# nipponjo/tts-arabic-pytorch

Measured on AMD Instinct MI355X. Metric: audio samples/sec (FastPitch+HiFi-GAN, synthetic 64-phoneme inputs), higher is better.
Workload: dtype f32

## Files before the change

tts-arabic-pytorch_amd/csrc/api.hip:

```cpp
#include <cerrno>
#include <cstdio>
#include <cstdlib>
#include <cstring>
#include <algorithm>
#include <atomic>
#include <mutex>
#include <string>
#include <vector>

#include "kernels.hpp"

namespace ttsamd {

static thread_local std::string g_err;

void set_error(const char* fmt, ...) {
    char buf[1024];
    va_list ap;
    va_start(ap, fmt);
    vsnprintf(buf, sizeof(buf), fmt, ap);
    va_end(ap);
    g_err = buf;
}

// ... 205 lines not shown
    unsigned v = __float_as_uint(r);
    v += 0x7fffu + ((v >> 16) & 1u);
    out[i] = (unsigned short)h;
    out[n + i] = (unsigned short)(v >> 16);
}

namespace {
struct OptDesc { const char* name; int kind; long long lo, hi; };
const OptDesc kOpts[OPT_COUNT] = {
#define TTS_OPT_DESC(name, kind, lo, hi) {"TTSAMD_" #name, kind, lo, hi},
    TTS_OPTIONS(TTS_OPT_DESC)
#undef TTS_OPT_DESC
};
std::atomic<const char*> g_opt[OPT_COUNT];
std::once_flag g_opt_once;
std::string g_opt_env_error;

bool opt_valid(const OptDesc& d, const char* v) {
    if (!v || !*v) return false;
    char* end = nullptr;
    errno = 0;
    const long long x = std::strtoll(v, &end, d.kind == 1 ? 16 : 10);
    if (!(errno == 0 && end != v && *end == '\0' && x >= d.lo && x <= d.hi)) return false;
    if (&d == &kOpts[OPT_WINO4] && (((x & 32) && !(x & 2)) || ((x & 64) && !(x & 4)) || ((x & 128) && !(x & 8)))) return false;
    return true;
}
void opt_init() {
    std::call_once(g_opt_once, [] {
        for (int i = 0; i < OPT_COUNT; ++i) {
            const char* e = std::getenv(kOpts[i].name);
            if (!e || !*e) continue;
            if (!opt_valid(kOpts[i], e)) {
                if (g_opt_env_error.empty()) {
                    char buf[256];
                    std::snprintf(buf, sizeof buf, "%s='%s' in the environment is not a valid value (%s in [%llx, %llx])", kOpts[i].name, e,
                                  kOpts[i].kind == 1 ? "hex mask" : "integer", kOpts[i].lo, kOpts[i].hi);
                    g_opt_env_error = buf;
                }
                continue;
            }
            g_opt[i].store(strdup(e), std::memory_order_release);
        }
    });
}
int opt_find(const char* name) {
    if (!name) return -1;
    for (int i = 0; i < OPT_COUNT; ++i)
// ... 844 lines not shown
```

tts-arabic-pytorch_amd/csrc/common.hpp:

```cpp
#pragma once
#include <hip/hip_runtime.h>
#include <stdint.h>
#include <atomic>
#include <cstdarg>
#include <cstdio>
#include <cstdlib>
#include <string>

#include "../../include/ttsamd.h"

namespace ttsamd {

void set_error(const char* fmt, ...);

#define TTS_CHECK_HIP(expr)                                                         \
    do {                                                                            \
        hipError_t e_ = (expr);                                                     \
        if (e_ != hipSuccess) {                                                     \
            ttsamd::set_error("%s failed: %s (%s:%d)", #expr, hipGetErrorString(e_), \
                              __FILE__, __LINE__);                                  \
            return TTSAMD_EHIP;                                                     \
        }                                                                           \
    } while (0)

// ... 7 lines not shown

#define TTS_TRY(expr)               \
    do {                            \
        int32_t rc_ = (expr);       \
        if (rc_ != 0) return rc_;   \
    } while (0)

inline int64_t align_up(int64_t x, int64_t a) { return (x + a - 1) / a * a; }

inline hipError_t lds_opt_in(const void* fn, int bytes, std::atomic<uint64_t>& done) {
    int dev = 0;
    hipError_t e = hipGetDevice(&dev);
    if (e != hipSuccess) return e;
    if (dev >= 0 && dev < 64 && ((done.load(std::memory_order_acquire) >> dev) & 1)) return hipSuccess;
    e = hipFuncSetAttribute(fn, hipFuncAttributeMaxDynamicSharedMemorySize, bytes);
    if (e == hipSuccess && dev >= 0 && dev < 64) done.fetch_or(1ull << dev, std::memory_order_release);
    return e;
}

#define TTS_OPTIONS(X)                                                                                     \
    X(HIFIGAN_STREAMS, 0, 0, 1)    \
    X(WINO, 0, 0, 1)                                              \
    X(WINO2, 0, 0, 31)             \
    X(WINO4, 0, 0, 255)            \
    X(FUSED_PAIR, 0, 0, 1)                   \
    X(FUSED2, 0, 0, 1)                                           \
    X(FUSED2_MASK, 1, 0, 0x1ff)               \
    X(FUSED2_MASK_N1, 1, 0, 0x1ff)          \
    X(FUSED2_WB, 0, 0, 2)                     \
    X(PAIR4, 0, 0, 2)              \
    X(CONVT, 0, 0, 1)                              \
    X(CONVT_WINO, 0, 0, 2)         \
    X(BFO, 0, 0, 1)                \
    X(BFO_CHAIN, 0, 0, 1)                           \
    X(BFO_CHAIN7, 0, 0, 1)                                 \
    X(BFO_FF, 0, 0, 1)                              \
    X(BFO_SPLITK, 0, 0, 1)                                              \
    X(BFO_SMALL_TILES, 0, 0, 1)            \
    X(BF16_ATTN, 0, 0, 1)                                         \
    X(BF16_PACKED_T, 0, 0, 1)                   \
    X(ATT_RA, 0, 1, 4)                             \
    X(ATT_SPLIT, 0, 0, 1)                      \
    X(XCD_W, 0, 0, 1)                            \
    X(XCD_WMAX_KB, 0, 0, 1 << 20)     \
    X(DEEP_SPLITK, 0, 0, 1)        \
    X(TACO_PERSISTENT, 0, 0, 2)    \
    X(TACO_SEG, 0, 8, 1 << 20)     \
// ... 93 lines not shown
                           int32_t mode, float div, float slope, int32_t ntw, hipStream_t stream, const float* w2_wino = nullptr,
                           const float* w1_wino = nullptr);
bool fused_pair4_supported(int32_t channels, int32_t k, int32_t dil, int32_t L, const float* x, const float* y);
int32_t launch_fused_pair4(int32_t channels, const float* x, float* y, const float* w1_wino4, const float* b1, const float* w2_wino4,
                           const float* b2, int32_t k, int32_t dil, const int64_t* lens, int32_t len_mul, int32_t L, int32_t batch,
                           int32_t mode, float div, float slope, hipStream_t stream, int32_t points = 6);
bool resblock2_conv_supported(int32_t channels, int32_t k, int32_t dil, int32_t L, const float* x, const float* y);
int32_t launch_resblock2_conv(int32_t channels, const float* x, float* y, const float* w, const float* b, int32_t k, int32_t dil,
                              const int64_t* lens, int32_t len_mul, int32_t L, int32_t batch, int32_t mode, float div, float slope,
                              hipStream_t stream);
bool resblock2_pair_supported(int32_t channels, int32_t k, int32_t d1, int32_t d2, int32_t L, const float* x, const float* y);
int32_t launch_resblock2_pair(int32_t channels, const float* x, float* y, const float* w1, const float* b1, const float* w2,
                              const float* b2, int32_t k, int32_t d1, int32_t d2, const int64_t* lens, int32_t len_mul, int32_t L,
                              int32_t batch, int32_t mode, float div, float slope, hipStream_t stream);
int wino_route(const ConvParams& p);
int32_t launch_wino(const ConvParams& p, hipStream_t stream);
void pack_wino_weight(const float* w, int cout, int cin, float* out);
int wino2_groups(int k);
int wino2_block_outputs(int coutp, int dil);
int32_t launch_wino2(const ConvParams& p, hipStream_t stream);
void pack_wino2_weight(const float* w, int cout, int cin, int k, float* out);
int wino4_groups(int k);
int wino44_groups(int k);
constexpr int kWino4Default = 255;
bool wino44_wanted(const ConvParams& p);
int wino4_block_outputs(int dil);
__host__ __device__ constexpr int wino4_pk_tuples(int n, int d) { return d * ((n + 4 * d - 1) / (4 * d)); }
__host__ __device__ constexpr int wino4_pk_tiles(int n, int d) { return (wino4_pk_tuples(n, d) + 63) / 64; }
__host__ __device__ constexpr int wino4_pk_col(int t, int d) { return (t / d) * 4 * d + t % d; }
__host__ __device__ constexpr int wino4_pk_q0(int tile, int d) { return (64 * tile / d) * 4 * d; }
__host__ __device__ constexpr int wino4_pk_r0(int tile, int d) { return 64 * tile % d; }
int wino4_ksplit(const ConvParams& p);
int32_t launch_splitk_reduce(const ConvParams& q, hipStream_t stream);
int32_t launch_wino4(const ConvParams& p, hipStream_t stream);
void wino4_filter_groups(const float* g, int k, float* o);
void pack_wino4_weight(const float* w, int cout, int cin, int k, float* out);
void wino44_filter_groups(const float* g, int k, float* o);
void pack_wino44_weight(const float* w, int cout, int cin, int k, float* out);
void pack_conv_weight(const float* w, int cout, int cin, int k, float* out);
void pack_convt_weight(const float* w, int cin, int cout, int kt, int u, int p, float* out);
inline int cout_padded(int cout) { return (int)align_up(cout, 32); }
void split_packed_bf16(const float* packed, int64_t n, uint16_t* out);
int32_t default_precision();

#ifdef __HIPCC__
template <int EXTRA = 0, bool PACKED = false>
__device__ __forceinline__ bool live_tile(const int64_t* __restrict__ lens, const int mul, const int n_max, const int tile_w,
// ... 37 lines not shown
```

tts-arabic-pytorch_amd/csrc/conv_wino4.hip:

```cpp
#include <cstdlib>
#include <cstring>

#include <algorithm>
#include <vector>

#include "conv_mfma_common.hpp"
#include "conv_row_epilogue.hpp"
#include "bfo.hpp"

namespace ttsamd {

typedef float w4_f32x4 __attribute__((ext_vector_type(4)));
typedef float w4_f32x2 __attribute__((ext_vector_type(2)));

template <int K, int NOCT_, int NSTAGE_, int PT_ = 6, int LP_ = 1, int CT_ = 0, int PK_ = 0>
struct Wino4Geo {
    static_assert(PK_ == 0 || LP_ == 2, "packed tiles: the strip kernels");
    static constexpr bool PT7 = PT_ == 7;
    static_assert(PT_ == 6 || (PT7 && (K == 7 || K == 11)), "seven-point groups: k = 7 / 11");
    static_assert(CT_ == 0 || (K == 3 && PT_ == 6 && LP_ == 1), "transposed conv: the k = 3 six-point form at dilation 1");
    static constexpr int WM = 2, WN = 2;
    static constexpr int NSF = K == 1 ? 0 : (K == 3 ? 1 : (K == 7 ? 2 : (PT7 ? 3 : 4)));
    static constexpr int NL = (!PT7 && (K == 7 || K == 1)) ? 1 : 0;
    static constexpr int GSF = PT7 ? 7 : 6;
    static constexpr int SSF = PT7 ? 4 : 3;
    static constexpr int NG = PT7 ? (K == 7 ? 13 : 20) : (K == 1 ? 4 : (K == 3 ? (CT_ ? 5 : 6) : (K == 7 ? 16 : 23)));
    static constexpr int NGQ = PT7 ? NG : ((NG + 1) & ~1);
    static constexpr bool WSHARE = K == 1;
    static constexpr int NGW = WSHARE ? 1 : NGQ;
    static constexpr int NPL = PT7 ? 7 : (NL ? 8 : (CT_ ? 5 : 6));
    static constexpr int NPOS = K == 1 ? 4 : (K == 3 ? (CT_ ? 5 : 6) : (K == 7 ? 10 : 14));
    static constexpr int NOCT = NOCT_, NSTAGE = NSTAGE_;
    static constexpr int NPH = PT7 ? ((K == 11 && LP_ == 2) ? 2 : 1) : (K == 11 ? 2 : 1);
    static constexpr int PH0 = PT7 ? 8 : 12;
    static constexpr int NGPM = NPH == 1 ? NG : 12;
    static_assert(NPH == 1 || (PH0 <= NGPM && NG - PH0 <= NGPM), "phase sizes");
    static constexpr int CO_BLK = WM * 32;
    static constexpr int NTUP = WN * 32;
    static constexpr int NT_BLK = 4 * NTUP;
    static constexpr int BUF4 = NOCT * 2 * NGPM * NTUP;
    static constexpr int PF = 4;
    static constexpr int NM = 4;
    __host__ __device__ static constexpr int glo(int ph) { return NPH == 1 ? 0 : PH0 * ph; }
// ... 13 lines not shown
    __host__ __device__ static constexpr int mlo(int ph) { return gfirst(glo(ph)); }
    __host__ __device__ static constexpr int mhi(int ph) {
        int m = 0;
        for (int g = glo(ph); g < glo(ph) + ngp(ph); ++g) m = glast(g) > m ? glast(g) : m;
        return m;
    }
    static_assert(mhi(NPH - 1) == NPOS - 1 && mlo(0) == 0, "the groups cover the window and nothing past it");
    __host__ __device__ static constexpr int npos(int ph) { return mhi(ph) - mlo(ph) + 1; }
    static constexpr int NPOSP = npos(0) > npos(NPH - 1) ? npos(0) : npos(NPH - 1);
    __host__ __device__ static constexpr int ngap(int ph) { return NOCT * ngp(ph) * NM; }
    __host__ __device__ static constexpr int sph(int ph) { return ((ph - (NSTAGE - 1)) % NPH + NPH) % NPH; }
    __host__ __device__ static constexpr int sgap(int ph) { return ngap(sph(ph)); }
    static constexpr int JSF = 10;
    __host__ __device__ static constexpr int sflo(int ph) { return glo(ph) / 7; }
    __host__ __device__ static constexpr bool inph(int ph, int g) { return g >= glo(ph) && g < glo(ph) + ngp(ph); }
    __host__ __device__ static constexpr int glast_ph(int ph) { return glo(ph) + ngp(ph) - 1; }
    __host__ __device__ static constexpr int nwj(int ph) {
        return PT7 ? JSF * (glast_ph(ph) / 7 - sflo(ph)) + (glast_ph(ph) % 7 == 0 ? 3 : JSF) : NOCT * ngp(ph);
    }
    static_assert(!PT7 || (NOCT == 1 && glo(0) % 7 <= 1 && glo(NPH - 1) % 7 <= 1 &&
                           (glast_ph(0) % 7 == 0 || glast_ph(0) % 7 >= 5) && glast_ph(NPH - 1) % 7 >= 5),
                  "seven-point phases: start on V0 / V1 of a sub-filter (the partial sums are formed per phase), end on V0 or the last row");
    __host__ __device__ static constexpr int fdiv4(int e) { return e >= 0 ? e / 4 : -((3 - e) / 4); }
    __host__ __device__ static constexpr int vlo(int ph) { return fdiv4(mlo(ph) - (K - 1) / 2); }
    __host__ __device__ static constexpr int nvec(int ph) { return fdiv4(mhi(ph) - (K - 1) / 2) - vlo(ph) + 1; }
    static constexpr int NVP = nvec(0) > nvec(NPH - 1) ? nvec(0) : nvec(NPH - 1);
    __host__ __device__ static constexpr int nljv(int ph) { return NOCT * 2 * nvec(ph); }
    static constexpr int DAV = (K == 3 || K == 1) ? 8 : 16;
    __host__ __device__ static constexpr int tw0v(int ph) { return DAV + 2 * nljv(ph); }
    __host__ __device__ static constexpr int wsv(int ph) { return (sgap(ph) - tw0v(ph)) / nwj(ph); }
    static_assert(LP_ != 1 || (wsv(0) >= 1 && wsv(NPH - 1) >= 1), "one write job per gap at most (vector loads)");
    __host__ __device__ static constexpr int strip_need(int d) {
        return 3 + (PK_ ? wino4_pk_col(d - 1 + 63, d) : wino4_pk_col(4 * 64 / (4 * d) * d - 1, d)) + (NPOS - 1) * d + 1;
    }
    static constexpr int RAWW = (PK_ && K == 11) ? 332 : 320;
    static_assert(RAWW % 4 == 0 && RAWW >= 256 && RAWW <= 512 && strip_need(3) <= RAWW && strip_need(5) <= RAWW, "the strip holds every tuple's window");
    static constexpr int NV2 = (RAWW - 256) / 4;
    static constexpr int NROW = 2 * NOCT;
    static constexpr int RAW_BYTES = 4 * (NROW * RAWW * 4 + 16);
    static constexpr int DAT = K == 7 ? 16 : (K == 11 ? 12 : 8);
    __host__ __device__ static constexpr int nrj(int ph) { return NROW * ((npos(ph) + 1) / 2); }
    __host__ __device__ static constexpr bool loads_in(int ph) { return ph == 0; }
    __host__ __device__ static constexpr int tr_r0(int ph) { return loads_in(ph) ? DAT + 2 * NROW : 0; }
    __host__ __device__ static constexpr int tw0t(int ph) { return tr_r0(ph) + nrj(ph) + 1; }
    __host__ __device__ static constexpr int wst(int ph) { return (sgap(ph) - tw0t(ph)) / nwj(ph); }
    static_assert(LP_ != 2 || (wst(0) >= 1 && wst(NPH - 1) >= 1), "one write job per gap at most (strip path)");
    static constexpr int QX = WSHARE ? 0 : (NOCT * ngq(0)) % PF;
    static constexpr int QMAIN = NOCT * ngq(0) - QX;
    static_assert(QX == 0 || (NPH == 1 && NOCT == 1 && QMAIN >= 2 * PF), "extra queue slots: one phase, one octet");
    static_assert((WSHARE ? NOCT : NOCT * ngq(NPH - 1)) % PF == 0 || QX != 0, "queue slots line up across steps");
    static_assert((size_t)NSTAGE * BUF4 * 16 + (LP_ == 2 ? RAW_BYTES : 0) <= 80 * 1024, "two blocks per CU");
    static_assert(NPH == 1 || NOCT == 1, "phases split an octet's groups");
};

// ... 19 lines not shown
        if (!wino4_pk_covers(n, d)) return false;
    return true;
}
static_assert(wino4_pk_covers_range(1, 1, 130, 1) && wino4_pk_covers_range(1, 131, 700, 13), "packed tiles, d = 1: rows of 1 .. 700 outputs");
static_assert(wino4_pk_covers_range(3, 1, 130, 1) && wino4_pk_covers_range(3, 131, 700, 13), "packed tiles, d = 3: rows of 1 .. 700 outputs");
static_assert(wino4_pk_covers_range(5, 1, 130, 1) && wino4_pk_covers_range(5, 131, 700, 13), "packed tiles, d = 5: rows of 1 .. 700 outputs");
static_assert(wino4_pk_covers_range(3, 1020, 1030, 1) && wino4_pk_covers_range(5, 1020, 1030, 1), "packed tiles: around 1028");
static_assert(wino4_pk_covers(1357, 3) && wino4_pk_covers(1357, 5) && wino4_pk_covers(2048, 3) && wino4_pk_covers(2048, 5), "packed tiles: long rows");
static_assert(wino4_pk_covers(28672, 3), "packed tiles, d = 3: a row of 28672");
static_assert(wino4_pk_covers(28672, 5), "packed tiles, d = 5: a row of 28672");
static_assert(wino4_pk_tiles(1028, 5) == 5 && wino4_pk_tuples(1028, 5) == 260 && wino4_pk_tuples(1028, 3) == 258, "packed tiles of a row of 1028");

template <int K, int NOCT_, int NSTAGE_, int EPI, int LP, int PT = 6>
__global__ __launch_bounds__(256, kConvMinWaves) void conv1d_wino4_f32(const ConvParams p) {
    extern __shared__ __attribute__((aligned(16))) float4 smem4[];
    constexpr int CTU = EPI == 5 ? 8 : (EPI == 6 ? 2 : 0);
    constexpr bool CT = CTU != 0;
    constexpr bool PK = EPI == 7;
    using G = Wino4Geo<K, NOCT_, NSTAGE_, PT, LP, CTU, PK ? 1 : 0>;
    constexpr bool PT7 = G::PT7;
    constexpr int WN = G::WN, NSF = G::NSF, NOCT = G::NOCT, NSTAGE = G::NSTAGE, NPL = G::NPL, NGPM = G::NGPM;
    constexpr int CO_BLK = G::CO_BLK, NTUP = G::NTUP, NT_BLK = G::NT_BLK, PF = G::PF;
    constexpr int NPH = G::NPH, NPOSP = G::NPOSP, NM = G::NM;
    constexpr bool D1 = LP == 1, TR = LP == 2;
    static_assert(D1 || TR, "window path");
    const int dil = D1 ? 1 : p.dil;
    const int nt_eff = wino4_tile(dil, NTUP), ntup_eff = nt_eff / 4;
    const int tiles_y = p.CoutP / CO_BLK;
    const int per_tile = tiles_y * p.ksplit;
    const unsigned sidx = blockIdx.x, xcd = sidx & 7u, u = sidx >> 3;
    const int yk = (int)(u % (unsigned)per_tile);
    const unsigned gt = (u / (unsigned)per_tile) * 8u + xcd;
    const int n_tiles_x = PK ? wino4_pk_tiles(p.Nout, dil) : (p.Nout + nt_eff - 1) / nt_eff;
    const int tile_w = PK ? 1 : nt_eff;
    int b = (int)(gt / (unsigned)n_tiles_x);
    int q0 = (int)(gt % (unsigned)n_tiles_x) * tile_w;
    if (p.compact) {
        int tile = 0;
        if (!live_tile<CT ? 1 : 0, PK>(p.lens_out, p.len_out_mul, p.Nout, nt_eff, p.batch, gt, b, tile, dil)) return;
        b = __builtin_amdgcn_readfirstlane(b);
        q0 = __builtin_amdgcn_readfirstlane(tile) * tile_w;
    } else if (b >= p.batch) {
        return;
    }
    int r0 = 0;
    if constexpr (PK) {
        r0 = wino4_pk_r0(q0, dil);
// ... 4 lines not shown
    const int ks = yk / tiles_y;
    const int co_blk0 = (yk - ks * tiles_y) * CO_BLK;
    int n_out = p.Nout;
    if constexpr (CT) {
        if (p.lens_out) {
            const int len = min(p.Lin, (int)p.lens_out[b] * p.len_out_mul);
            n_out = len > 0 ? len + 1 : 0;
        }
    } else {
        if (p.lens_out) n_out = min(n_out, (int)p.lens_out[b] * p.len_out_mul);
    }
    if (q0 >= n_out) return;
    int in_len = p.Lin;
    if (p.lens_in) in_len = min(in_len, (int)p.lens_in[b] * p.len_in_mul);

    const int x_cs = p.x_cs, CoutP = p.CoutP;
    const int chunks_all = p.Cin / (8 * NOCT);
    const int c_beg = (int)((int64_t)ks * chunks_all / p.ksplit), n_chunks = (int)((int64_t)(ks + 1) * chunks_all / p.ksplit);
    const int n_groups = (p.Cin / 8) * G::NGW;
    const float* __restrict__ xb = p.x + (int64_t)b * p.x_bs;
    const float in_slope = p.in_slope;

    constexpr bool REG = EPI >= 3, RES = EPI == 3;
    static_assert(!REG || ((LP == 1 || PK) && K != 1), "register epilogue: dilation 1 or the packed strip form, k = 3 / 7 / 11");
    static_assert(!PK || LP == 2, "packed tiles: the strip kernels");
    static_assert(EPI <= 7 && (!CT || K == 3), "epilogues 0, 3, 4, 7 and the transposed conv's 5 / 6 (k = 3 form)");
    float ep_bias = 0.f;
    if constexpr (!REG) {
        if (tid < CO_BLK && p.bias) ep_bias = p.bias[min(co_blk0 + tid, p.Cout - 1)];
    }

    const int kk = lane >> 5, l31 = lane & 31;
    const int pe = wn * 32 + l31;
    const int col_e = PK ? wino4_pk_col(r0 + pe, dil) : (dil == 1 ? 4 * pe : (pe / dil) * 4 * dil + pe % dil);
    f32x16 acc[NPL];
#pragma unroll
    for (int g = 0; g < NPL; ++g)
#pragma unroll
        for (int r = 0; r < 16; ++r) acc[g][r] = 0.f;
    const int ep_row0 = REG ? co_blk0 + __builtin_amdgcn_readfirstlane(wm) * 32 : 0;
    const int ep_voff = (q0 + col_e < n_out ? q0 + col_e : 0) * 4;
    const int ep_rrow = ep_row0 + 4 * kk;
    const bfo_i4 ep_rs = bfo_rsrc(RES ? p.res + (int64_t)b * p.r_bs : nullptr, RES ? (unsigned)p.Cout * (unsigned)p.r_cs * 4u : 0u);
    const bfo_i4 ep_bs = bfo_rsrc(p.bias, (REG && p.bias) ? (unsigned)p.Cout * 4u : 0u);
    w4_f32x4 rq[RES ? 16 : 1], bsq[REG ? 4 : 1];
    constexpr int EP_T0 = RES ? 16 : 0;
#define TTS_EPLOAD_JOB(T)                                                                            \
// ... 4 lines not shown
            bsq[REG ? (T) - EP_T0 : 0] = __builtin_bit_cast(w4_f32x4, bfo_ld16(ep_bs, (ep_rrow + 8 * ((T) - EP_T0)) * 4, 0, 0)); \
    }

    const bfo_i4 wrs = bfo_rsrc(K == 1 ? p.w : (PT7 ? p.w_wino44 : p.w_wino4), (unsigned)n_groups * 2u * (unsigned)CoutP * 16u);
    const int wv = (kk * CoutP + co_blk0 + wm * 32 + l31) * 16;
    const int wstep = 2 * CoutP * 16, wlast = (n_groups - 1) * wstep;
    int wso = c_beg * NOCT * G::NGW * wstep;
    w4_f32x4 aq[PF + G::QX];
    if constexpr (G::QX == 0) {
#pragma unroll
        for (int g = 0; g < PF; ++g) {
            aq[g] = __builtin_bit_cast(w4_f32x4, bfo_ld16(wrs, wv, wso, 0));
            wso = min(wso + wstep, wlast);
        }
    } else {
#pragma unroll
        for (int g = 0; g < PF + G::QX; ++g)
            aq[g] = __builtin_bit_cast(w4_f32x4, bfo_ld16(wrs, wv, min(wso + (g < PF ? g : G::QMAIN + g - PF) * wstep, wlast), 0));
    }

    const int sh = __builtin_amdgcn_readfirstlane((tid >> 7) & 1), skk = __builtin_amdgcn_readfirstlane((tid >> 6) & 1);
    w4_f32x2 sx[D1 ? 1 : NOCT][D1 ? 1 : NPOSP];
    w4_f32x4 sv[D1 ? NOCT : 1][2][D1 ? G::NVP : 1];
    w4_f32x2 ta[NOCT], tb[NOCT];
    w4_f32x2 tf[PT7 ? 5 : 1], te[PT7 ? 4 : 1], td[PT7 ? 3 : 1], th[PT7 ? 2 : 1];
    const int spe = PK ? r0 + lane : min(lane, ntup_eff - 1);
    const int xw0 = (q0 + 4 * lane) * 4;
    constexpr int pad_c = (K - 1) / 2;
    const int ch_off = (4 * sh + skk) * x_cs;

#define TTS_VJOB_IDX(PH, J)                                                                          \
        const int nv_ = G::nvec(PH);                                                                 \
        const int ol_ = (J) / (2 * nv_), pp_ = ((J) / nv_) % 2, vi_ = (J) % nv_;
#define TTS_VLOAD_JOB(PH, J, XSO)                                                                    \
    {                                                                                                \
        TTS_VJOB_IDX(PH, J)                                                                          \
        const bfo_i4 xrs_ = bfo_rsrc(xb + ((XSO) + ch_off + (8 * ol_ + 2 * pp_) * x_cs), (unsigned)in_len * 4u);     \
        sv[ol_][pp_][vi_] = __builtin_bit_cast(w4_f32x4, bfo_ld16(xrs_, xw0 + 16 * (G::vlo(PH) + vi_), 0, 0));      \
    }
#define TTS_VACT_JOB(PH, A)                                                                          \
    {                                                                                                \
        TTS_VJOB_IDX(PH, (A) / 2)                                                                    \
        if ((A) % 2 == 0) {                                                                          \
            sv[ol_][pp_][vi_].x = bfo_lrelu(sv[ol_][pp_][vi_].x, in_slope);                          \
            sv[ol_][pp_][vi_].y = bfo_lrelu(sv[ol_][pp_][vi_].y, in_slope);                          \
        } else {                                                                                     \
            sv[ol_][pp_][vi_].z = bfo_lrelu(sv[ol_][pp_][vi_].z, in_slope);                          \
            sv[ol_][pp_][vi_].w = bfo_lrelu(sv[ol_][pp_][vi_].w, in_slope);                          \
        }                                                                                            \
    }
    float* const strip = reinterpret_cast<float*>(smem4 + NSTAGE * G::BUF4) + wid * (G::NROW * G::RAWW + 4);
    const int tr_a = (q0 - pad_c * dil) & ~3;
    const int tr_off = q0 + (dil == 1 ? 4 * spe : (spe / dil) * 4 * dil + spe % dil) - pad_c * dil - tr_a;
    w4_f32x4 rv[TR ? G::NROW : 1][2];
#define TTS_TLOAD_JOB(J, XSO)                                                                        \
    {                                                                                                \
        const int pp_ = (J) / 2, vs_ = (J) % 2;                                                      \
        const bfo_i4 xrs_ = bfo_rsrc(xb + ((XSO) + ch_off + (8 * (pp_ / 2) + 2 * (pp_ % 2)) * x_cs), (unsigned)in_len * 4u); \
        const int v_ = lane + 64 * vs_;                                                              \
        rv[pp_][vs_] = __builtin_bit_cast(w4_f32x4, bfo_ld16(xrs_, (vs_ == 1 && lane >= G::NV2) ? BFO_OOB : (tr_a + 4 * v_) * 4, 0, 0)); \
    }
#define TTS_TSTORE_JOB(J)                                                                            \
    {                                                                                                \
        const int pp_ = (J) / 2, vs_ = (J) % 2;                                                      \
        w4_f32x4 a_ = rv[pp_][vs_];                                                                  \
        a_.x = bfo_lrelu(a_.x, in_slope); a_.y = bfo_lrelu(a_.y, in_slope);                          \
        a_.z = bfo_lrelu(a_.z, in_slope); a_.w = bfo_lrelu(a_.w, in_slope);                          \
        const int v_ = lane + 64 * vs_;                                                              \
        float* dst_ = (vs_ == 1 && lane >= G::NV2) ? strip + G::NROW * G::RAWW : strip + pp_ * G::RAWW + 4 * v_;    \
        *reinterpret_cast<w4_f32x4*>(dst_) = a_;                                                     \
    }
#define TTS_TREAD_JOB(PH, J)                                                                         \
    {                                                                                                \
        const int npr_ = (G::npos(PH) + 1) / 2;                                                      \
        const int pp_ = (J) / npr_, jp_ = (J) % npr_;                                                \
        const float* src_ = strip + pp_ * G::RAWW + tr_off + (G::mlo(PH) + 2 * jp_) * dil;           \
        sx[pp_ / 2][2 * jp_][pp_ % 2] = src_[0];                                                     \
        if (2 * jp_ + 1 < G::npos(PH)) sx[pp_ / 2][2 * jp_ + 1][pp_ % 2] = src_[dil];                \
    }
#define TTS_SXV(M) (w4_f32x2{sv[ol_][0][G::fdiv4((M) - pad_c) - G::vlo(PH_)][((M) - pad_c) - 4 * G::fdiv4((M) - pad_c)],     \
                             sv[ol_][1][G::fdiv4((M) - pad_c) - G::vlo(PH_)][((M) - pad_c) - 4 * G::fdiv4((M) - pad_c)]})
#define TTS_SX(M) (D1 ? TTS_SXV(M) : sx[D1 ? 0 : ol_][D1 ? 0 : (M) - G::mlo(PH_)])
#define TTS_WRITE_JOB(PH, J, WR)                                                                     \
    {                                                                                                \
        const int PH_ = (PH);                                                                        \
        const int ol_ = PT7 ? 0 : (J) / G::ngp(PH_), gl_ = (J) % G::ngp(PH_), g_ = G::glo(PH_) + gl_;                          \
        w4_f32x2 v2;                                                                                 \
        if constexpr (PT7) {                                                                         \
             \
            const int sf_ = G::sflo(PH_) + (J) / G::JSF, kd_ = (J) % G::JSF, s4 = 4 * sf_, g0_ = 7 * sf_;                      \
            const bool v0_ = G::inph(PH_, g0_), tap4_ = g0_ + 6 < G::NG;                             \
            int row_ = -1;                                                                           \
            if (kd_ == 0) {                         \
                if (v0_) tf[0] = sf_ > G::sflo(PH_) ? tf[4] : TTS_SX(s4 + 2) - 4.f * TTS_SX(s4);    \
                tf[1] = TTS_SX(s4 + 3) - 4.f * TTS_SX(s4 + 1);                                       \
                tf[2] = TTS_SX(s4 + 4) - 4.f * TTS_SX(s4 + 2);                                       \
            } else if (kd_ == 1) {                                                                   \
                tf[3] = TTS_SX(s4 + 5) - 4.f * TTS_SX(s4 + 3);                                       \
                if (v0_) te[0] = tf[0] - 2.f * tf[1];                                                \
            } else if (kd_ == 2) {                                                                   \
                te[2] = tf[2] - 2.f * tf[3];                                                         \
                if (v0_) { v2 = te[2] - te[0]; row_ = 0; }                                           \
            } else if (kd_ == 3) {                                                                   \
                te[1] = tf[1] - 2.f * tf[2];                                                         \
                v2 = te[1] + te[2]; row_ = 1;                                                        \
// ... 34 lines not shown
                v2 = ta[ol_] + tb[ol_];                                                              \
            } else if (i_ == 4) v2 = ta[ol_] - tb[ol_];                                              \
            else v2 = 4.f * TTS_SX(s3 + 1) + (TTS_SX(s3 + 5 < G::NPOS ? s3 + 5 : s3) - 5.f * TTS_SX(s3 + 3));           \
        } else {                                                                                     \
            v2 = TTS_SX(3 * NSF + (g_ - 6 * NSF));                                                   \
        }                                                                                            \
        if constexpr (!PT7) (WR)[2 * ((ol_ * 2 * NGPM + gl_) * NTUP)] = v2;                          \
    }

    const float4* sB = smem4 + kk * NGPM * NTUP + wn * 32 + l31;
    w4_f32x2* sW = reinterpret_cast<w4_f32x2*>(smem4 + skk * NGPM * NTUP + lane) + sh;
    float4 bq[2];

    {
#pragma unroll
        for (int st = 0; st < NSTAGE - 1; ++st) {
            const int ph = st % NPH;
            const int xso = min(c_beg + st / NPH, n_chunks - 1) * 8 * NOCT * x_cs;
            if constexpr (D1) {
#pragma unroll
                for (int J = 0; J < G::nljv(ph); ++J) TTS_VLOAD_JOB(ph, J, xso)
#pragma unroll
                for (int J = 0; J < 2 * G::nljv(ph); ++J) TTS_VACT_JOB(ph, J)
            } else {
                if (G::loads_in(ph)) {
#pragma unroll
                    for (int J = 0; J < 2 * G::NROW; ++J) TTS_TLOAD_JOB(J, xso)
#pragma unroll
                    for (int J = 0; J < 2 * G::NROW; ++J) TTS_TSTORE_JOB(J)
                }
#pragma unroll
                for (int J = 0; J < G::nrj(ph); ++J) TTS_TREAD_JOB(ph, J)
            }
            w4_f32x2* wr = sW + 2 * st * G::BUF4;
#pragma unroll
            for (int J = 0; J < G::nwj(ph); ++J) TTS_WRITE_JOB(ph, J, wr)
        }
    }
    __syncthreads();
    bq[0] = sB[0];

    int stage = 0;
#define TTS_CHUNK_STEPS(LAST, C) \
        _Pragma("unroll")                                                                                                                                    \
        for (int ph = 0; ph < NPH; ++ph) {                                                                                                                   \
            const bool peel = (LAST) && ph == NPH - 1;                                                                                                       \
// ... 20 lines not shown
                    aq[qs] = __builtin_bit_cast(w4_f32x4, bfo_ld16(wrs, wv, wso, 0));                                                                        \
                    wso = min(wso + wstep, wlast);                                                                                                           \
                }                                                                                                                                            \
                if (gl >= G::ngp(ph)) continue;                                                     \
                const int r = ol * G::ngp(ph) + gl;                                                                \
                const int cur = r & 1, nxt = cur ^ 1;                                                                                                        \
                const int plane = G::plane(G::glo(ph) + gl);                                                                                                 \
                                                    \
                if (r + 1 < NOCT * G::ngp(ph)) bq[nxt] = rd[(((r + 1) / G::ngp(ph)) * 2 * NGPM + (r + 1) % G::ngp(ph)) * NTUP];                              \
                else if (NSTAGE >= 3 && !peel) bq[nxt] = sB[sn * G::BUF4];        \
                __builtin_amdgcn_sched_barrier(0);                                                                                                           \
                const float bv[4] = {bq[cur].x, bq[cur].y, bq[cur].z, bq[cur].w};                                                                            \
        _Pragma("unroll")                                                                                                                                    \
                for (int m = 0; m < NM; ++m) {                                                                                                               \
                    acc[plane] = __builtin_amdgcn_mfma_f32_32x32x2f32(a4[m], bv[m], acc[plane], 0, 0, 0);                                                    \
                                   \
                                                                                             \
                    const int t = r * NM + m;                                                                                                                \
                    if (peel) {                                                                                                                              \
                        TTS_EPLOAD_JOB(t)                                                                                                                    \
                    } else if constexpr (D1) {                                                                                                               \
                        if (t < G::nljv(tph)) TTS_VLOAD_JOB(tph, t, xso)                                                                                     \
                        if (t >= G::DAV && t - G::DAV < 2 * G::nljv(tph)) TTS_VACT_JOB(tph, t - G::DAV)                                                      \
                        if (t >= G::tw0v(tph) && (t - G::tw0v(tph)) % G::wsv(tph) == 0 &&                                                                    \
                            (t - G::tw0v(tph)) / G::wsv(tph) < G::nwj(tph))                                                                                  \
                            TTS_WRITE_JOB(tph, (t - G::tw0v(tph)) / G::wsv(tph), wr)                                                                         \
                    } else {                                                                                                                                 \
                        if (G::loads_in(tph) && t < 2 * G::NROW) TTS_TLOAD_JOB(t, xso)                                                                       \
                        if (G::loads_in(tph) && t >= G::DAT && t < G::DAT + 2 * G::NROW) TTS_TSTORE_JOB(t - G::DAT)                                          \
                        if (t >= G::tr_r0(tph) && t - G::tr_r0(tph) < G::nrj(tph)) TTS_TREAD_JOB(tph, t - G::tr_r0(tph))                                     \
                        if (t >= G::tw0t(tph) && (t - G::tw0t(tph)) % G::wst(tph) == 0 && (t - G::tw0t(tph)) / G::wst(tph) < G::nwj(tph))                    \
                            TTS_WRITE_JOB(tph, (t - G::tw0t(tph)) / G::wst(tph), wr)                                                                         \
                    }                                                                                                                                        \
                    __builtin_amdgcn_sched_barrier(0);                                                                                                       \
                }                                                                                                                                            \
            }                                                                                                                                                \
            if (peel) break;                                                                                                                                 \
            __syncthreads();                                                                                                                                 \
            if (NSTAGE < 3) bq[0] = sB[sn * G::BUF4];                                      \
            else if ((NOCT * G::ngp(ph)) % 2 != 0) bq[0] = bq[1];                                                                                            \
            stage = stage_next;                                                                                                                              \
        }
    for (int c = c_beg; c < n_chunks - (REG ? 1 : 0); ++c) {
        TTS_CHUNK_STEPS(false, c)
    }
    if constexpr (REG) {
        const int c = n_chunks - 1;
        TTS_CHUNK_STEPS(true, c)
    }
#undef TTS_CHUNK_STEPS
#undef TTS_EPLOAD_JOB
#undef TTS_TLOAD_JOB
#undef TTS_TSTORE_JOB
#undef TTS_TREAD_JOB
#undef TTS_VLOAD_JOB
#undef TTS_VACT_JOB
#undef TTS_VJOB_IDX
#undef TTS_SXV
#undef TTS_SX
#undef TTS_WRITE_JOB

#define TTS_OUT_QUAD(R)                                                                              \
        const float s12 = acc[1][R] + acc[2][R], d12 = acc[1][R] - acc[2][R];                        \
        const float s34 = acc[3][R] + acc[4][R], d34 = acc[3][R] - acc[4][R];                        \
        float y0 = acc[0][R] + s12 + s34;                                                            \
        float y1 = d12 + 2.f * d34;                                                                  \
        float y2 = s12 + 4.f * s34;                                                                  \
        float y3 = d12 + 8.f * d34 + acc[PT7 ? 6 : 5][R];                                            \
        if constexpr (NSF == 0) { y0 = acc[0][R]; y1 = 0.f; y2 = 0.f; y3 = acc[5][R]; }               \
        if constexpr (PT7) {                                                                   \
            y0 += acc[5][R];                                                                         \
            y1 += 0.5f * acc[5][R];                                                                  \
            y2 += 0.25f * acc[5][R];                                                                 \
            y3 += 0.125f * acc[5][R];                                                                \
        } else if constexpr (NPL == 8) {                                                             \
            y1 += acc[6][R];                                                                         \
            y2 += acc[7][R];                                                                         \
        }
// ... 193 lines not shown
    static_assert(EPI < 3 || lds == ring + strip, "register epilogue: the ring (and the strip) set the LDS size");
    static std::atomic<uint64_t> lds_done{0};
    const auto kern = conv1d_wino4_f32<K, NOCT, NSTAGE, EPI, LP, PT>;
    TTS_CHECK_HIP(lds_opt_in((const void*)kern, (int)lds, lds_done));
    const int nt = wino4_tile(p.dil, G::NTUP);
    ConvParams q = p;
    q.ksplit = EPI == 0 ? wino4_ksplit(p) : 1;
    note_conv_launch(PK ? (PT == 7 ? 8 : 7) : (PT == 7 ? 4 : 3), q.ksplit);
    const int64_t n_tiles = (int64_t)(PK ? wino4_pk_tiles(p.Nout, p.dil) : (p.Nout + nt - 1) / nt) * p.batch;
    const int64_t n_blocks = ((n_tiles + 7) / 8) * 8 * (p.CoutP / G::CO_BLK) * q.ksplit;
    TTS_REQUIRE(n_blocks < ((int64_t)1 << 31), "wino4: %lld blocks", (long long)n_blocks);
    dim3 grid((unsigned)n_blocks, 1, 1);
    q.compact = compact_order(p.lens_out, p.batch) ? 1 : 0;
    hipLaunchKernelGGL(kern, grid, dim3(256), lds, stream, q);
    TTS_CHECK_HIP(hipGetLastError());
    if (q.ksplit > 1) return launch_splitk_reduce(q, stream);
    return 0;
}

static bool wino4_packed_wanted(const ConvParams& p) {
    return ((int)opt_int(OPT_WINO4, kWino4Default) & 128) != 0 && p.dil != 1 && p.res == nullptr && p.mode == 0 && wino4_ksplit(p) == 1;
}

template <int K, int NOCT, int NSTAGE>
static int32_t launch_wino4_cfg(const ConvParams& p, hipStream_t stream) {
    if (p.dil == 1) {
        if (wino4_ksplit(p) != 1) return launch_wino4_epi<K, NOCT, NSTAGE, 0, 1>(p, stream);
        if (p.res != nullptr) return launch_wino4_epi<K, NOCT, NSTAGE, 3, 1>(p, stream);
        return launch_wino4_epi<K, NOCT, NSTAGE, 4, 1>(p, stream);
    }
    if (wino4_packed_wanted(p)) return launch_wino4_epi<K, NOCT, 2, 7, 2>(p, stream);
    return launch_wino4_epi<K, NOCT, 2, 0, 2>(p, stream);
}

template <int K>
static int32_t launch_wino44_cfg(const ConvParams& p, hipStream_t stream) {
    if (p.dil == 1) {
        if (wino4_ksplit(p) != 1) return launch_wino4_epi<K, 1, 2, 0, 1, 7>(p, stream);
        if (p.res != nullptr) return launch_wino4_epi<K, 1, 2, 3, 1, 7>(p, stream);
        return launch_wino4_epi<K, 1, 2, 4, 1, 7>(p, stream);
    }
    if (wino4_packed_wanted(p)) return launch_wino4_epi<K, 1, 2, 7, 2, 7>(p, stream);
    return launch_wino4_epi<K, 1, 2, 0, 2, 7>(p, stream);
}

bool wino44_wanted(const ConvParams& p) {
    if (p.w_wino44 == nullptr || (p.K != 7 && p.K != 11)) return false;
    return ((int)opt_int(OPT_WINO4, kWino4Default) & (p.K == 7 ? 32 : 64)) != 0;
}
// ... 2 lines not shown
    if (wino44_wanted(p)) return p.K == 7 ? launch_wino44_cfg<7>(p, stream) : launch_wino44_cfg<11>(p, stream);
    if (p.K == 1) return launch_wino4_epi<1, 4, 2, 0, 1>(p, stream);
    if (p.K == 3) return launch_wino4_cfg<3, 2, 3>(p, stream);
    if (p.K == 7) return launch_wino4_cfg<7, 1, 2>(p, stream);
    if (p.K == 11) return launch_wino4_cfg<11, 1, 3>(p, stream);
    set_error("wino4: kernel size %d not built (1, 3, 7, 11)", p.K);
    return TTSAMD_EINVAL;
}

int wino4_block_outputs(int dil) { return wino4_tile(dil, 64); }

bool convt_wino_packable(int cin, int cout, int u) { return (u == 2 || u == 8) && cin >= 16 && cin % 16 == 0 && cout >= 1 && (u * cout) % 64 == 0; }

bool convt_wino_supported(const ConvParams& p, const float* w_wino, const float* bias_wino) {
    const int u = p.n_phase;
    return w_wino != nullptr && bias_wino != nullptr && p.precision == 0 && convt_wino_packable(p.Cin, p.Cout, u) && p.K == 2 && p.dil == -1 &&
           p.phase_p * 2 == u && p.y_ts == u && p.res == nullptr && p.mode == 0 && p.scale == nullptr && p.relu_out == 0 &&
           !p.x_packed && !p.y_packed && p.in_slope >= 0.f && p.in_slope <= 1.f && p.Lin == p.Nout &&
           (p.x_cs & 3) == 0 && (p.x_bs & 3) == 0 && ((uintptr_t)p.x & 15) == 0 &&
           (p.y_cs & 3) == 0 && (p.y_bs & 3) == 0 && ((uintptr_t)p.y & 15) == 0 &&
           (int64_t)p.Lin * 4 + 64 < ((int64_t)1 << 31) && (int64_t)p.Cout * p.y_cs * 4 < ((int64_t)1 << 31);
}

template <int U>
static int32_t launch_convt_wino_u(const ConvParams& p, const float* w_wino, const float* bias_wino, hipStream_t stream) {
    constexpr int EPI = U == 8 ? 5 : 6;
    using G = Wino4Geo<3, 2, 3, 6, 1, U>;
    constexpr size_t lds = (size_t)G::NSTAGE * G::BUF4 * sizeof(float4);
    static_assert(lds <= 80 * 1024, "two blocks per CU");
    static std::atomic<uint64_t> lds_done{0};
    const auto kern = conv1d_wino4_f32<3, 2, 3, EPI, 1, 6>;
    TTS_CHECK_HIP(lds_opt_in((const void*)kern, (int)lds, lds_done));
    ConvParams q = p;
    q.w_wino4 = w_wino; q.bias = bias_wino;
    q.Cout = U * p.Cout; q.CoutP = q.Cout;
    q.Nout = p.Lin + 1;
    q.K = 3; q.dil = 1; q.pad = 1; q.n_phase = 1; q.ksplit = 1;
    const int64_t n_tiles = (int64_t)((q.Nout + G::NT_BLK - 1) / G::NT_BLK) * p.batch;
    const int64_t n_blocks = ((n_tiles + 7) / 8) * 8 * (q.CoutP / G::CO_BLK);
    TTS_REQUIRE(n_blocks < ((int64_t)1 << 31), "convt wino: %lld blocks", (long long)n_blocks);
    q.compact = compact_order(p.lens_out, p.batch) ? 1 : 0;
    hipLaunchKernelGGL(kern, dim3((unsigned)n_blocks, 1, 1), dim3(256), lds, stream, q);
    TTS_CHECK_HIP(hipGetLastError());
    return 0;
}

int32_t launch_convt_wino(const ConvParams& p, const float* w_wino, const float* bias_wino, hipStream_t stream) {
    TTS_REQUIRE(convt_wino_supported(p, w_wino, bias_wino), "convt wino: unsupported geometry");
    if (p.Nout <= 0) return 0;
    conv_log("convt_wino", 2, p.Cin, p.Cout, p.Nout, p.batch, 0, 0, p.len_out_mul, p.lens_out != nullptr, p.n_phase);
    note_conv_launch(6, 1);
    return p.n_phase == 8 ? launch_convt_wino_u<8>(p, w_wino, bias_wino, stream) : launch_convt_wino_u<2>(p, w_wino, bias_wino, stream);
}

void pack_convt_wino_weight(const float* w, const float* bias, int cin, int cout, int u, float* out_w, float* out_bias) {
    const int rows = u * cout;
    std::vector<float> t((size_t)rows * cin * 3);
    for (int ci = 0; ci < cin; ++ci)
        for (int co = 0; co < cout; ++co)
            for (int j = 0; j < u; ++j) {
                const float* g = w + ((int64_t)ci * cout + co) * 2 * u;
                float* d = t.data() + ((int64_t)(co * u + j) * cin + ci) * 3;
                d[0] = g[j + u]; d[1] = g[j]; d[2] = 0.f;
            }
    pack_wino4_weight(t.data(), rows, cin, 3, out_w);
    for (int r = 0; r < rows; ++r) out_bias[r] = bias ? bias[r / u] : 0.f;
}

int wino4_ksplit(const ConvParams& p) {
    const int bo = wino4_block_outputs(p.dil);
    const int64_t blocks = (int64_t)((p.Nout + bo - 1) / bo) * (p.CoutP / 64) * p.batch;
    constexpr int sk_blocks = 192, sk_target = 224;
    if (blocks >= sk_blocks || p.splitk_ws == nullptr) return 1;
    const int n_chunks = p.Cin / (p.K == 1 ? 32 : (p.K == 3 ? 16 : 8));
    const int64_t per = (int64_t)p.batch * p.Cout * p.Nout;
// ... 53 lines not shown
```

Before: 79.82 million.

## Add own-vector window path for k=3 dilation-1 Winograd conv using DPP edge exchange

Adds a new window mode (LP=3) for the k=3 six-point Winograd conv at dilation 1. Each lane loads only its own float4 vector. The neighbouring edge elements come from cross-lane DPP shifts, and only lanes 0 and 63 issue an extra scalar edge load. This replaces the multi-vector overlapping loads per lane, cutting global load traffic and registers, at the cost of DPP ops and a longer pipeline delay (DAV). It is enabled by default through the new WINO4 bit 256, which also covers the transposed-conv upsamplers.

```diff
diff --git a/profiles/r35/k3_classes.py b/profiles/r35/k3_classes.py
--- /dev/null
+++ b/profiles/r35/k3_classes.py
@@ -0,0 +1,48 @@
+import csv
+import re
+import sys
+from collections import defaultdict
+
+NAMES = {(3, 3, 7936): 'HiFi-GAN c2, C = 128 (residual)', (3, 4, 7936): 'HiFi-GAN c1 d = 1, C = 128', (3, 3, 2048): 'HiFi-GAN c2, C = 256 (residual)',
+         (3, 4, 2048): 'HiFi-GAN c1 d = 1, C = 256', (3, 3, 384): 'conv-FF 1536 -> 384 (residual)', (3, 4, 1536): 'conv-FF 384 -> 1536',
+         (3, 5, 8192): 'upsampler u = 8, 512 -> 256', (3, 5, 2048): 'upsampler u = 8, 256 -> 128', (3, 6, 8000): 'upsampler u = 2, 128 -> 64',
+         (3, 6, 7968): 'upsampler u = 2, 64 -> 32'}
+
+
+def classes(path):
+    d = defaultdict(lambda: [0, 0])
+    other = 0
+    with open(path) as f:
+        for r in csv.DictReader(f):
+            dur = int(r['End_Timestamp']) - int(r['Start_Timestamp'])
+            m = re.search(r'conv1d_wino4_f32<(\d+), (\d+), (\d+), (\d+), (\d+), (\d+)>', r['Kernel_Name'])
+            if not m:
+                other += dur
+                continue
+            k, noct, nst, epi, lp, pt = map(int, m.groups())
+            key = (k, noct, nst, epi, pt, 'strip' if lp == 2 else 'd = 1', int(r['Grid_Size_X']) // int(r['Workgroup_Size_X']))
+            d[key][0] += 1
+            d[key][1] += dur
+    return d, other
+
+
+a, oa = classes(sys.argv[1])
+b, ob = classes(sys.argv[2])
+print(f'{"k":>3} {"EPI":>3} {"groups":>6} {"window":>6} {"blocks":>6} {"calls":>5} {"us parent":>10} {"us tree":>9} {"ratio":>6}  class')
+sums = {'k = 3, dilation 1 (changed)': [0, 0], 'control (k = 7 / 11, k = 1, strip)': [0, 0]}
+lo, hi = 9.0, 0.0
+for key in sorted(set(a) | set(b), key=lambda t: (t[0] != 3 or t[5] != 'd = 1', t[0], t[5], t[3], t[6])):
+    ca, da = a.get(key, (0, 0))
+    cb, db = b.get(key, (0, 0))
+    changed = key[0] == 3 and key[5] == 'd = 1'
+    s = sums['k = 3, dilation 1 (changed)' if changed else 'control (k = 7 / 11, k = 1, strip)']
+    s[0] += da
+    s[1] += db
+    ua, ub = (da / ca / 1e3 if ca else float('nan')), (db / cb / 1e3 if cb else float('nan'))
+    if not changed and ca and cb:
+        lo, hi = min(lo, ub / ua), max(hi, ub / ua)
+    print(f'{key[0]:3d} {key[3]:3d} {"seven" if key[4] == 7 else "six":>6} {key[5]:>6} {key[6]:6d} {max(ca, cb):5d} {ua:10.1f} {ub:9.1f} {ub / ua:6.3f}  '
+          f'{NAMES.get((key[0], key[3], key[6]), "") if changed else ""}')
+for name, (da, db) in sums.items():
+    print(f'{name}: {da / 1e6:.3f} -> {db / 1e6:.3f} ms over the trace ({db / da:.4f}x)')
+print(f'control classes: {lo:.3f}x .. {hi:.3f}x; every other kernel: {oa / 1e6:.2f} -> {ob / 1e6:.2f} ms (whole trace)')
diff --git a/tts-arabic-pytorch_amd/csrc/api.hip b/tts-arabic-pytorch_amd/csrc/api.hip
--- a/tts-arabic-pytorch_amd/csrc/api.hip
+++ b/tts-arabic-pytorch_amd/csrc/api.hip
@@ -251,7 +251,7 @@
     errno = 0;
     const long long x = std::strtoll(v, &end, d.kind == 1 ? 16 : 10);
     if (!(errno == 0 && end != v && *end == '\0' && x >= d.lo && x <= d.hi)) return false;
-    if (&d == &kOpts[OPT_WINO4] && (((x & 32) && !(x & 2)) || ((x & 64) && !(x & 4)) || ((x & 128) && !(x & 8)))) return false;
+    if (&d == &kOpts[OPT_WINO4] && (((x & 32) && !(x & 2)) || ((x & 64) && !(x & 4)) || ((x & 128) && !(x & 8)) || ((x & 256) && !(x & 1)))) return false;
     return true;
 }
 void opt_init() {
diff --git a/tts-arabic-pytorch_amd/csrc/common.hpp b/tts-arabic-pytorch_amd/csrc/common.hpp
--- a/tts-arabic-pytorch_amd/csrc/common.hpp
+++ b/tts-arabic-pytorch_amd/csrc/common.hpp
@@ -53,7 +53,7 @@
     X(HIFIGAN_STREAMS, 0, 0, 1)    \
     X(WINO, 0, 0, 1)                                              \
     X(WINO2, 0, 0, 31)             \
-    X(WINO4, 0, 0, 255)            \
+    X(WINO4, 0, 0, 511)            \
     X(FUSED_PAIR, 0, 0, 1)                   \
     X(FUSED2, 0, 0, 1)                                           \
     X(FUSED2_MASK, 1, 0, 0x1ff)               \
@@ -193,7 +193,7 @@
 void pack_wino2_weight(const float* w, int cout, int cin, int k, float* out);
 int wino4_groups(int k);
 int wino44_groups(int k);
-constexpr int kWino4Default = 255;
+constexpr int kWino4Default = 511;
 bool wino44_wanted(const ConvParams& p);
 int wino4_block_outputs(int dil);
 __host__ __device__ constexpr int wino4_pk_tuples(int n, int d) { return d * ((n + 4 * d - 1) / (4 * d)); }
diff --git a/tts-arabic-pytorch_amd/csrc/conv_wino4.hip b/tts-arabic-pytorch_amd/csrc/conv_wino4.hip
--- a/tts-arabic-pytorch_amd/csrc/conv_wino4.hip
+++ b/tts-arabic-pytorch_amd/csrc/conv_wino4.hip
@@ -18,7 +18,9 @@
     static_assert(PK_ == 0 || LP_ == 2, "packed tiles: the strip kernels");
     static constexpr bool PT7 = PT_ == 7;
     static_assert(PT_ == 6 || (PT7 && (K == 7 || K == 11)), "seven-point groups: k = 7 / 11");
-    static_assert(CT_ == 0 || (K == 3 && PT_ == 6 && LP_ == 1), "transposed conv: the k = 3 six-point form at dilation 1");
+    static_assert(CT_ == 0 || (K == 3 && PT_ == 6 && (LP_ == 1 || LP_ == 3)), "transposed conv: the k = 3 six-point form at dilation 1");
+    static constexpr bool SW = LP_ == 3;
+    static_assert(!SW || (K == 3 && PT_ == 6), "own-vector window: the k = 3 six-point form at dilation 1");
     static constexpr int WM = 2, WN = 2;
     static constexpr int NSF = K == 1 ? 0 : (K == 3 ? 1 : (K == 7 ? 2 : (PT7 ? 3 : 4)));
     static constexpr int NL = (!PT7 && (K == 7 || K == 1)) ? 1 : 0;
@@ -78,14 +80,16 @@
                            (glast_ph(0) % 7 == 0 || glast_ph(0) % 7 >= 5) && glast_ph(NPH - 1) % 7 >= 5),
                   "seven-point phases: start on V0 / V1 of a sub-filter (the partial sums are formed per phase), end on V0 or the last row");
     __host__ __device__ static constexpr int fdiv4(int e) { return e >= 0 ? e / 4 : -((3 - e) / 4); }
-    __host__ __device__ static constexpr int vlo(int ph) { return fdiv4(mlo(ph) - (K - 1) / 2); }
-    __host__ __device__ static constexpr int nvec(int ph) { return fdiv4(mhi(ph) - (K - 1) / 2) - vlo(ph) + 1; }
+    __host__ __device__ static constexpr int vlo(int ph) { return SW ? 0 : fdiv4(mlo(ph) - (K - 1) / 2); }
+    __host__ __device__ static constexpr int nvec(int ph) { return SW ? 1 : fdiv4(mhi(ph) - (K - 1) / 2) - vlo(ph) + 1; }
     static constexpr int NVP = nvec(0) > nvec(NPH - 1) ? nvec(0) : nvec(NPH - 1);
     __host__ __device__ static constexpr int nljv(int ph) { return NOCT * 2 * nvec(ph); }
-    static constexpr int DAV = (K == 3 || K == 1) ? 8 : 16;
-    __host__ __device__ static constexpr int tw0v(int ph) { return DAV + 2 * nljv(ph); }
+    __host__ __device__ static constexpr int nej(int ph) { return SW ? NOCT * 2 : 0; }
+    static constexpr int DAV = SW ? (CT_ ? 12 : 20) : ((K == 3 || K == 1) ? 8 : 16);
+    __host__ __device__ static constexpr int tw0v(int ph) { return DAV + 2 * nljv(ph) + nej(ph); }
     __host__ __device__ static constexpr int wsv(int ph) { return (sgap(ph) - tw0v(ph)) / nwj(ph); }
-    static_assert(LP_ != 1 || (wsv(0) >= 1 && wsv(NPH - 1) >= 1), "one write job per gap at most (vector loads)");
+    static_assert((LP_ != 1 && LP_ != 3) || (wsv(0) >= 1 && wsv(NPH - 1) >= 1), "one write job per gap at most (vector loads)");
+    static_assert(!SW || nljv(0) + nej(0) <= DAV, "own-vector window: every load is issued before the first activation");
     __host__ __device__ static constexpr int strip_need(int d) {
         return 3 + (PK_ ? wino4_pk_col(d - 1 + 63, d) : wino4_pk_col(4 * 64 / (4 * d) * d - 1, d)) + (NPOS - 1) * d + 1;
     }
@@ -151,7 +155,8 @@
     constexpr int WN = G::WN, NSF = G::NSF, NOCT = G::NOCT, NSTAGE = G::NSTAGE, NPL = G::NPL, NGPM = G::NGPM;
     constexpr int CO_BLK = G::CO_BLK, NTUP = G::NTUP, NT_BLK = G::NT_BLK, PF = G::PF;
     constexpr int NPH = G::NPH, NPOSP = G::NPOSP, NM = G::NM;
-    constexpr bool D1 = LP == 1, TR = LP == 2;
+    constexpr bool SW = LP == 3;
+    constexpr bool D1 = LP == 1 || SW, TR = LP == 2;
     static_assert(D1 || TR, "window path");
     const int dil = D1 ? 1 : p.dil;
     const int nt_eff = wino4_tile(dil, NTUP), ntup_eff = nt_eff / 4;
@@ -202,7 +207,7 @@
     const float in_slope = p.in_slope;
 
     constexpr bool REG = EPI >= 3, RES = EPI == 3;
-    static_assert(!REG || ((LP == 1 || PK) && K != 1), "register epilogue: dilation 1 or the packed strip form, k = 3 / 7 / 11");
+    static_assert(!REG || ((D1 || PK) && K != 1), "register epilogue: dilation 1 or the packed strip form, k = 3 / 7 / 11");
     static_assert(!PK || LP == 2, "packed tiles: the strip kernels");
     static_assert(EPI <= 7 && (!CT || K == 3), "epilogues 0, 3, 4, 7 and the transposed conv's 5 / 6 (k = 3 form)");
     float ep_bias = 0.f;
@@ -253,10 +258,12 @@
     const int sh = __builtin_amdgcn_readfirstlane((tid >> 7) & 1), skk = __builtin_amdgcn_readfirstlane((tid >> 6) & 1);
     w4_f32x2 sx[D1 ? 1 : NOCT][D1 ? 1 : NPOSP];
     w4_f32x4 sv[D1 ? NOCT : 1][2][D1 ? G::NVP : 1];
+    float se[SW ? NOCT : 1][2], sl[SW ? NOCT : 1][2], sr[SW ? NOCT : 1][2];
     w4_f32x2 ta[NOCT], tb[NOCT];
     w4_f32x2 tf[PT7 ? 5 : 1], te[PT7 ? 4 : 1], td[PT7 ? 3 : 1], th[PT7 ? 2 : 1];
     const int spe = PK ? r0 + lane : min(lane, ntup_eff - 1);
     const int xw0 = (q0 + 4 * lane) * 4;
+    const int xe0 = lane == 0 ? (q0 - 1) * 4 : ((!CT && lane == 63) ? (q0 + NT_BLK) * 4 : BFO_OOB);
     constexpr int pad_c = (K - 1) / 2;
     const int ch_off = (4 * sh + skk) * x_cs;
 
@@ -280,6 +287,20 @@
             sv[ol_][pp_][vi_].w = bfo_lrelu(sv[ol_][pp_][vi_].w, in_slope);                          \
         }                                                                                            \
     }
+#define TTS_ELOAD_JOB(J, XSO)                                                                        \
+    {                                                                                                \
+        const int ol_ = (J) / 2, pp_ = (J) % 2;                                                      \
+        const bfo_i4 xrs_ = bfo_rsrc(xb + ((XSO) + ch_off + (8 * ol_ + 2 * pp_) * x_cs), (unsigned)in_len * 4u);     \
+        se[SW ? ol_ : 0][pp_] = bfo_ld4f(xrs_, xe0, 0, 0);                                           \
+    }
+#define TTS_EACT_JOB(J)                                                                              \
+    {                                                                                                \
+        const int ol_ = SW ? (J) / 2 : 0, pp_ = (J) % 2;                                             \
+        const int e_ = __builtin_bit_cast(int, bfo_lrelu(se[ol_][pp_], in_slope));                   \
+        sl[ol_][pp_] = __builtin_bit_cast(float, __builtin_amdgcn_update_dpp(e_, __builtin_bit_cast(int, (float)sv[ol_][pp_][0].w), 0x138, 0xf, 0xf, false));    \
+        if constexpr (!CT)                                                                           \
+            sr[ol_][pp_] = __builtin_bit_cast(float, __builtin_amdgcn_update_dpp(e_, __builtin_bit_cast(int, (float)sv[ol_][pp_][0].x), 0x130, 0xf, 0xf, false)); \
+    }
     float* const strip = reinterpret_cast<float*>(smem4 + NSTAGE * G::BUF4) + wid * (G::NROW * G::RAWW + 4);
     const int tr_a = (q0 - pad_c * dil) & ~3;
     const int tr_off = q0 + (dil == 1 ? 4 * spe : (spe / dil) * 4 * dil + spe % dil) - pad_c * dil - tr_a;
@@ -311,7 +332,10 @@
     }
 #define TTS_SXV(M) (w4_f32x2{sv[ol_][0][G::fdiv4((M) - pad_c) - G::vlo(PH_)][((M) - pad_c) - 4 * G::fdiv4((M) - pad_c)],     \
                              sv[ol_][1][G::fdiv4((M) - pad_c) - G::vlo(PH_)][((M) - pad_c) - 4 * G::fdiv4((M) - pad_c)]})
-#define TTS_SX(M) (D1 ? TTS_SXV(M) : sx[D1 ? 0 : ol_][D1 ? 0 : (M) - G::mlo(PH_)])
+#define TTS_SXW(M) ((M) == 0 ? w4_f32x2{sl[SW ? ol_ : 0][0], sl[SW ? ol_ : 0][1]}                     \
+                             : ((M) == 5 ? w4_f32x2{sr[SW ? ol_ : 0][0], sr[SW ? ol_ : 0][1]}        \
+                                         : w4_f32x2{sv[ol_][0][0][((M) - 1) & 3], sv[ol_][1][0][((M) - 1) & 3]}))
+#define TTS_SX(M) (SW ? TTS_SXW(M) : (D1 ? TTS_SXV(M) : sx[D1 ? 0 : ol_][D1 ? 0 : (M) - G::mlo(PH_)]))
 #define TTS_WRITE_JOB(PH, J, WR)                                                                     \
     {                                                                                                \
         const int PH_ = (PH);                                                                        \
@@ -392,6 +416,12 @@
                 for (int J = 0; J < G::nljv(ph); ++J) TTS_VLOAD_JOB(ph, J, xso)
 #pragma unroll
                 for (int J = 0; J < 2 * G::nljv(ph); ++J) TTS_VACT_JOB(ph, J)
+                if constexpr (SW) {
+#pragma unroll
+                    for (int J = 0; J < G::nej(ph); ++J) TTS_ELOAD_JOB(J, xso)
+#pragma unroll
+                    for (int J = 0; J < G::nej(ph); ++J) TTS_EACT_JOB(J)
+                }
             } else {
                 if (G::loads_in(ph)) {
 #pragma unroll
@@ -458,6 +488,10 @@
                     } else if constexpr (D1) {                                                                                                               \
                         if (t < G::nljv(tph)) TTS_VLOAD_JOB(tph, t, xso)                                                                                     \
                         if (t >= G::DAV && t - G::DAV < 2 * G::nljv(tph)) TTS_VACT_JOB(tph, t - G::DAV)                                                      \
+                        if constexpr (SW) {                                                                                                                  \
+                            if (t >= G::nljv(tph) && t - G::nljv(tph) < G::nej(tph)) TTS_ELOAD_JOB(t - G::nljv(tph), xso)                                    \
+                            if (t >= G::DAV + 2 * G::nljv(tph) && t - G::DAV - 2 * G::nljv(tph) < G::nej(tph)) TTS_EACT_JOB(t - G::DAV - 2 * G::nljv(tph))   \
+                        }                                                                                                                                    \
                         if (t >= G::tw0v(tph) && (t - G::tw0v(tph)) % G::wsv(tph) == 0 &&                                                                    \
                             (t - G::tw0v(tph)) / G::wsv(tph) < G::nwj(tph))                                                                                  \
                             TTS_WRITE_JOB(tph, (t - G::tw0v(tph)) / G::wsv(tph), wr)                                                                         \
@@ -490,6 +524,9 @@
 #undef TTS_TSTORE_JOB
 #undef TTS_TREAD_JOB
 #undef TTS_VLOAD_JOB
+#undef TTS_ELOAD_JOB
+#undef TTS_EACT_JOB
+#undef TTS_SXW
 #undef TTS_VACT_JOB
 #undef TTS_VJOB_IDX
 #undef TTS_SXV
@@ -729,9 +766,18 @@
     return ((int)opt_int(OPT_WINO4, kWino4Default) & 128) != 0 && p.dil != 1 && p.res == nullptr && p.mode == 0 && wino4_ksplit(p) == 1;
 }
 
+static bool wino4_own_vector_wanted() { return ((int)opt_int(OPT_WINO4, kWino4Default) & 256) != 0; }
+
 template <int K, int NOCT, int NSTAGE>
 static int32_t launch_wino4_cfg(const ConvParams& p, hipStream_t stream) {
     if (p.dil == 1) {
+        if constexpr (K == 3) {
+            if (wino4_own_vector_wanted()) {
+                if (wino4_ksplit(p) != 1) return launch_wino4_epi<K, NOCT, NSTAGE, 0, 3>(p, stream);
+                if (p.res != nullptr) return launch_wino4_epi<K, NOCT, NSTAGE, 3, 3>(p, stream);
+                return launch_wino4_epi<K, NOCT, NSTAGE, 4, 3>(p, stream);
+            }
+        }
         if (wino4_ksplit(p) != 1) return launch_wino4_epi<K, NOCT, NSTAGE, 0, 1>(p, stream);
         if (p.res != nullptr) return launch_wino4_epi<K, NOCT, NSTAGE, 3, 1>(p, stream);
         return launch_wino4_epi<K, NOCT, NSTAGE, 4, 1>(p, stream);
@@ -780,14 +826,14 @@
            (int64_t)p.Lin * 4 + 64 < ((int64_t)1 << 31) && (int64_t)p.Cout * p.y_cs * 4 < ((int64_t)1 << 31);
 }
 
-template <int U>
+template <int U, int LP>
 static int32_t launch_convt_wino_u(const ConvParams& p, const float* w_wino, const float* bias_wino, hipStream_t stream) {
     constexpr int EPI = U == 8 ? 5 : 6;
-    using G = Wino4Geo<3, 2, 3, 6, 1, U>;
+    using G = Wino4Geo<3, 2, 3, 6, LP, U>;
     constexpr size_t lds = (size_t)G::NSTAGE * G::BUF4 * sizeof(float4);
     static_assert(lds <= 80 * 1024, "two blocks per CU");
     static std::atomic<uint64_t> lds_done{0};
-    const auto kern = conv1d_wino4_f32<3, 2, 3, EPI, 1, 6>;
+    const auto kern = conv1d_wino4_f32<3, 2, 3, EPI, LP, 6>;
     TTS_CHECK_HIP(lds_opt_in((const void*)kern, (int)lds, lds_done));
     ConvParams q = p;
     q.w_wino4 = w_wino; q.bias = bias_wino;
@@ -808,7 +854,9 @@
     if (p.Nout <= 0) return 0;
     conv_log("convt_wino", 2, p.Cin, p.Cout, p.Nout, p.batch, 0, 0, p.len_out_mul, p.lens_out != nullptr, p.n_phase);
     note_conv_launch(6, 1);
-    return p.n_phase == 8 ? launch_convt_wino_u<8>(p, w_wino, bias_wino, stream) : launch_convt_wino_u<2>(p, w_wino, bias_wino, stream);
+    if (wino4_own_vector_wanted())
+        return p.n_phase == 8 ? launch_convt_wino_u<8, 3>(p, w_wino, bias_wino, stream) : launch_convt_wino_u<2, 3>(p, w_wino, bias_wino, stream);
+    return p.n_phase == 8 ? launch_convt_wino_u<8, 1>(p, w_wino, bias_wino, stream) : launch_convt_wino_u<2, 1>(p, w_wino, bias_wino, stream);
 }
 
 void pack_convt_wino_weight(const float* w, const float* bias, int cin, int cout, int u, float* out_w, float* out_bias) {
```

Result: no change. 80.39 million, median of 6 (+0.7%).
